# google-research/nerf-from-image

Hardware: AMD Instinct MI355X
Metric: rendered rays/sec (128x128, 64+64 samples) (higher is better)
Workload: dtype f32 (decoder MLP operands split-fp16 hi+lo, 22 bits; strict fp32: config.value_mlp_exact_fp32)

## Files before the change

### include/nfi_hip.h

```cpp
#ifndef NFI_HIP_H
#define NFI_HIP_H

#include <stddef.h>
#include <stdint.h>

#ifdef __cplusplus
extern "C" {
#endif

typedef void* nfi_stream_t;

typedef enum nfi_status {
  NFI_OK = 0,
  NFI_ERR_INVALID_ARGUMENT = -1,
  NFI_ERR_UNSUPPORTED = -2,
  NFI_ERR_WORKSPACE_TOO_SMALL = -3,
  NFI_ERR_LAUNCH = -4
} nfi_status;

enum { NFI_PLANE_CHANNELS = 32, NFI_HIDDEN = 64, NFI_MAX_ATTENTION = 14, NFI_MAX_SAMPLES = 128 };
enum { NFI_MAX_SAMPLES_SINGLE_PASS = 512 };

enum { NFI_TEXEL_F32 = 0, NFI_TEXEL_BF16 = 1, NFI_TEXEL_F16 = 2 };
enum { NFI_TEXELS_PLANAR = 0, NFI_TEXELS_INTERLEAVED = 1 };
// ... 239 lines not shown
  float* semantics;
  float* ray_origins; float* ray_directions; float* near_plane; float* far_plane; uint8_t* hit;
  float* t_coarse; float* sigma_coarse; float* rgb_coarse;
  float* t_fine; float* sigma_fine; float* rgb_fine;
  float* t_sorted; float* weights; int32_t* perm;
  void* workspace; size_t workspace_bytes;
  int skip_missed_rays;
  void* event_start; void* event_stop;
  int tuning;
  void* profile_cycles;
  const float* ray_features;
  float termination_eps;
  int texel_layout;
  void* clock_probe;
  int row_offset; int full_height;
  float* stash_t; float* stash_sigma; float* stash_rgb;
  int rays_ready;
  float* coords;
  float* normals;
} nfi_render_args;
size_t nfi_render_workspace_bytes(int64_t n_rays);
int nfi_render_fwd(const nfi_render_args* a, nfi_stream_t stream);
const char* nfi_render_kernel_name(const nfi_render_args* a);
int nfi_render_setup(const nfi_render_args* a, nfi_stream_t stream);

typedef struct nfi_pnp_args {
  int n_images; int height; int width;
  const float* coords;
  const float* mask;
  float mask_threshold;
  int n_focal; const float* focal_proposals;
  int refine_iterations;
  void* workspace; size_t workspace_bytes;
  float* world2cam;
  float* focal;
  float* error;
} nfi_pnp_args;
size_t nfi_pnp_workspace_bytes(int n_images, int n_focal);
int nfi_pose_pnp(const nfi_pnp_args* a, nfi_stream_t stream);

typedef struct nfi_pose_args {
  int n_images, camera_flipped, normalize_q;
  const float* q; const float* t2; const float* s; const float* z0;
  float* cam2world; float* focal;
  const float* g_cam2world; const float* g_focal;
  float* g_q; float* g_t2; float* g_s; float* g_z0;
// ... 165 lines not shown
```

### nerf_from_image_amd/csrc/nfi_render_host.inc

```

struct RenderWorkspaceHeader {
  uint32_t reduce[3];
  uint32_t counter;
  uint32_t pad[12];
  uint32_t xcd_counter[8][16];
};
static_assert(sizeof(RenderWorkspaceHeader) == 64 + 8 * 64 && offsetof(RenderWorkspaceHeader, xcd_counter) == 64,
              "the render workspace header is read from Python and by the kernels' 16-dword counter stride");

static size_t render_workspace_prefix_bytes(int64_t n_rays) {
  size_t n = (size_t)n_rays;
  return sizeof(RenderWorkspaceHeader) + n * 8 * sizeof(float) + ((n + 63) & ~(size_t)63);
}

static size_t render_workspace_table_offset(int64_t n_rays) {
  return render_workspace_prefix_bytes(n_rays) + kRayBlocks * sizeof(RayPartial);
}

extern "C" size_t nfi_render_workspace_bytes(int64_t n_rays) {
  return render_workspace_table_offset(n_rays) + ((size_t)n_rays / 64) * sizeof(uint32_t);
}

struct BlockGeometry { int shift, ok; uint32_t bw, bh, n_blocks; };
static BlockGeometry render_block_geometry(const nfi_render_args* a) {
  BlockGeometry g;
  const int both = a->width | a->height;
  g.shift = (both & 31) == 0 ? 5 : ((both & 15) == 0 ? 4 : 3);
  const int side = 1 << g.shift;
  g.ok = (a->width % side == 0) && (a->height % side == 0) ? 1 : 0;
  g.bw = (uint32_t)a->width >> g.shift; g.bh = (uint32_t)a->height >> g.shift;
  g.n_blocks = g.bw * g.bh * (uint32_t)a->n_scenes;
  return g;
}

__device__ __forceinline__ uint32_t count_wide_hits(const uint8_t* p, int bytes) {
  uint32_t c = 0;
  if (bytes == 16 && (reinterpret_cast<uintptr_t>(p) & 15) == 0) {
    const uint4 v = *reinterpret_cast<const uint4*>(p);
    c = __popc(v.x & 0x02020202u) + __popc(v.y & 0x02020202u) + __popc(v.z & 0x02020202u) + __popc(v.w & 0x02020202u);
  } else if ((reinterpret_cast<uintptr_t>(p) & 3) == 0) {
    for (int i = 0; i < bytes; i += 4) c += __popc(*reinterpret_cast<const uint32_t*>(p + i) & 0x02020202u);
  } else {
    for (int i = 0; i < bytes; ++i) c += (p[i] >> 1) & 1u;
  }
  return c;
}

struct BlockTableParams { const uint8_t* hit; uint32_t* table; int shift, width, hw; uint32_t bw, bps, n_blocks, groups; };

__global__ __launch_bounds__(256) void raygen_finish_kernel(const RayPartial* __restrict__ partial, int n_partials,
                                                            RenderWorkspaceHeader* __restrict__ head, BlockTableParams t) {
  if (blockIdx.x != 0) {
    __shared__ uint32_t s_part[256], s_count[16];
    const uint32_t G = blockIdx.x - 1, i = threadIdx.x >> 4, sub = threadIdx.x & 15u;
    const uint32_t b = 16u * G + i, scene = b / t.bps, bb = b - scene * t.bps, by = bb / t.bw, bx = bb - by * t.bw;
    const uint8_t* base = t.hit + (size_t)scene * (size_t)t.hw + (size_t)(by << t.shift) * (size_t)t.width + (bx << t.shift);
    const int side = 1 << t.shift, cw = side < 16 ? side : 16, per_row = side / cw;
    uint32_t c = 0;
    for (int ch = (int)sub; ch < side * per_row; ch += 16)
      c += count_wide_hits(base + (size_t)(ch / per_row) * (size_t)t.width + (ch % per_row) * cw, cw);
    s_part[threadIdx.x] = c;
    __syncthreads();
    if (threadIdx.x < 16) {
      uint32_t sum = 0;
      for (int j = 0; j < 16; ++j) sum += s_part[threadIdx.x * 16 + j];
      s_count[threadIdx.x] = sum;
    }
    __syncthreads();
    if (threadIdx.x < 16) {
      const uint32_t me = threadIdx.x, mine = s_count[me];
      uint32_t r = 0;
      for (uint32_t j = 0; j < 16; ++j) r += (s_count[j] > mine || (s_count[j] == mine && j < me)) ? 1u : 0u;
      const uint32_t pair = r < 8 ? r : 15u - r, x = (pair + G) & 7u;
      t.table[16u * G + (r < 8 ? 0u : 8u) + x] = 16u * G + me;
    }
    return;
  }
  uint32_t kmin = 0u, kmax = 0u, cnt = 0u;
  for (int i = threadIdx.x; i < n_partials; i += blockDim.x) {
    const RayPartial p = partial[i];
    kmin = p.kmin > kmin ? p.kmin : kmin;
    kmax = p.kmax > kmax ? p.kmax : kmax;
    cnt += p.cnt;
  }
  block_reduce_keys(kmin, kmax, cnt);
  uint32_t* cells = reinterpret_cast<uint32_t*>(head);
  for (int i = 3 + threadIdx.x; i < (int)(sizeof(RenderWorkspaceHeader) / sizeof(uint32_t)); i += blockDim.x) cells[i] = 0u;
  if (threadIdx.x == 0) { head->reduce[0] = kmin; head->reduce[1] = kmax; head->reduce[2] = cnt; }
  for (uint32_t g = 16u * t.groups + threadIdx.x; g < t.n_blocks; g += blockDim.x) t.table[g] = g;
}

struct RenderWorkspace {
  RenderWorkspaceHeader* head; float* ro; float* rd; float* near_raw; float* far_raw; uint8_t* hit; RayPartial* partial; uint32_t* block_table; int64_t n;
};

static int render_carve(const nfi_render_args* a, RenderWorkspace& w) {
  REQUIRE(a && a->cam2world && a->workspace, "render: null pointer");
  REQUIRE(a->n_scenes > 0 && a->height > 0 && a->width > 0, "render: bad image shape");
  const int64_t n = (int64_t)a->n_scenes * a->height * a->width;
  if (a->workspace_bytes < nfi_render_workspace_bytes(n)) return fail(NFI_ERR_WORKSPACE_TOO_SMALL, "render: workspace too small");
  w.n = n;
  w.head = reinterpret_cast<RenderWorkspaceHeader*>(a->workspace);
  float* rays = reinterpret_cast<float*>(w.head + 1);
  w.ro = a->ray_origins ? a->ray_origins : rays;
  w.rd = a->ray_directions ? a->ray_directions : rays + 3 * n;
  w.near_raw = rays + 6 * n;
  w.far_raw = rays + 7 * n;
  w.hit = a->hit ? a->hit : reinterpret_cast<uint8_t*>(rays + 8 * n);
  w.partial = reinterpret_cast<RayPartial*>(reinterpret_cast<char*>(a->workspace) + render_workspace_prefix_bytes(n));
  w.block_table = reinterpret_cast<uint32_t*>(reinterpret_cast<char*>(a->workspace) + render_workspace_table_offset(n));
  return NFI_OK;
}

static int render_setup(const nfi_render_args* a, const RenderWorkspace& w, hipStream_t s) {
  const int full_h = a->full_height > 0 ? a->full_height : a->height;
  REQUIRE(a->row_offset >= 0 && a->row_offset + a->height <= full_h, "render: row window outside the image");
  CameraParams cam{a->cam2world, a->focal, a->bbox, a->focal ? a->center : nullptr, full_h, a->width, 1, a->height, a->row_offset};
  RaygenOut rout{w.ro, w.rd, w.near_raw, w.far_raw, w.hit, w.partial, a->scene_range};
  const int blocks = (int)std::min<int64_t>((w.n + 255) / 256, kRayBlocks);
  hipLaunchKernelGGL(raygen_kernel, dim3((unsigned)blocks), dim3(256), 0, s, cam, a->n_scenes, rout);
  const BlockGeometry g = render_block_geometry(a);
  const uint32_t n_table = g.ok ? g.n_blocks : (uint32_t)(w.n / 64), groups = g.ok ? g.n_blocks / 16 : 0u;
  const BlockTableParams t{w.hit, w.block_table, g.shift, a->width, a->height * a->width, g.bw, g.bw * g.bh, n_table, groups};
  hipLaunchKernelGGL(raygen_finish_kernel, dim3(1 + groups), dim3(256), 0, s, w.partial, blocks, w.head, t);
  return NFI_OK;
}

extern "C" int nfi_render_setup(const nfi_render_args* a, nfi_stream_t stream) {
  RenderWorkspace w;
  int rc = render_carve(a, w);
  if (rc) return rc;
  rc = render_setup(a, w, (hipStream_t)stream);
  if (rc) return rc;
  return check_launch("render_setup");
}

struct RenderFlags { bool stash, debug_tap, any_tap, strict, term, extra; };

static RenderFlags render_flags(const nfi_render_args* a) {
  RenderFlags f;
  f.stash = a->stash_t || a->stash_sigma || a->stash_rgb;
  f.debug_tap = a->t_coarse || a->sigma_coarse || a->rgb_coarse || a->t_fine || a->sigma_fine || a->rgb_fine ||
                a->t_sorted || a->weights || a->perm || a->near_plane || a->far_plane;
  f.any_tap = f.debug_tap || f.stash;
  f.strict = (a->tuning & NFI_TUNING_EXACT_FP32_MLP) != 0;
  f.term = a->termination_eps > 0.0f;
  f.extra = a->semantics || a->coords || a->normals;
// ... 39 lines not shown
  RenderKernelParams k;
  memset(&k, 0, sizeof(k));
  k.n_scenes = a->n_scenes; k.hw = a->height * a->width; k.S = a->n_samples;
  k.fine = a->fine_sampling; k.white = a->white_background; k.scene_range = a->scene_range;
  k.ro = w.ro; k.rd = w.rd; k.near_raw = w.near_raw; k.far_raw = w.far_raw; k.hit = w.hit; k.reduce = w.head->reduce;
  k.texels = a->texels; k.res = a->plane_res; k.layout = a->texel_layout; k.image = a->decoder_image; k.A = a->n_attention; k.att = a->attention_values;
  k.use_sdf = a->use_sdf; k.beta = a->beta; k.alpha = a->alpha;
  k.noise_c = a->noise_coarse; k.noise_f = a->noise_fine; k.noise_f_stride = a->noise_fine_row_stride;
  k.rgb = a->rgb; k.depth = a->depth; k.mask = a->mask;
  k.near_plane = a->near_plane; k.far_plane = a->far_plane;
  k.t_coarse = a->t_coarse; k.sigma_coarse = a->sigma_coarse; k.rgb_coarse = a->rgb_coarse;
  k.t_fine = a->t_fine; k.sigma_fine = a->sigma_fine; k.rgb_fine = a->rgb_fine;
  k.tap_stride = a->n_samples;
  if (f.stash) {
    k.tap_stride = (a->fine_sampling ? 2 : 1) * a->n_samples; k.stash = 1;
    k.t_coarse = a->stash_t; k.sigma_coarse = a->stash_sigma; k.rgb_coarse = a->stash_rgb;
    if (a->fine_sampling) {
      k.t_fine = a->stash_t + a->n_samples;
      k.sigma_fine = a->stash_sigma + a->n_samples;
      k.rgb_fine = a->stash_rgb + 3 * (size_t)a->n_samples;
    }
  }
  k.t_sorted = a->t_sorted; k.weights = a->weights; k.perm = a->perm;
  k.skip_missed = (a->skip_missed_rays && !f.debug_tap) ? 1 : 0;

  k.counter = &w.head->counter;
  k.xcd_counter = &w.head->xcd_counter[0][0];
  k.width = a->width;
  k.fetch_batch = 2;
  const BlockGeometry geo = render_block_geometry(a);
  k.xcd_block_shift = geo.shift;
  k.xcd_blocks = (!(a->tuning & NFI_TUNING_SINGLE_WORK_COUNTER) && geo.ok) ? 1 : 0;
  k.block_table = (k.xcd_blocks && !(a->tuning & NFI_TUNING_XCD_BLOCKS_IN_ORDER)) ? w.block_table : nullptr;
  const uint32_t bw = geo.bw, bh = geo.bh;
  k.div_scene_rays = make_fastdiv((uint32_t)k.hw * (uint32_t)std::max(a->views_per_scene, 1));
  k.div_bw = make_fastdiv(bw > 0 ? bw : 1u);
  k.div_bps = make_fastdiv(bw * bh > 0 ? bw * bh : 1u);
  k.tile_order = (!(a->tuning & NFI_TUNING_SCANLINE_ORDER) && (a->width % 8 == 0) && (a->height % 8 == 0)) ? 1 : 0;
  k.prof = (unsigned long long*)a->profile_cycles;
  k.xray = a->ray_features;
  k.clock_probe = reinterpret_cast<unsigned long long*>(a->clock_probe);
  k.term_eps = a->termination_eps;
  k.semantics = a->semantics; k.coords = a->coords; k.normals = a->normals;
  return k;
}

using RenderKernel = void (*)(RenderKernelParams);
struct RenderLaunch {
  RenderKernel kernel;
  const char* name;
  int occ;
  size_t max_lds;
  int (*raise_lds)(size_t, const char*);
};
static constexpr char kFwdFamily[] = "render_fwd_kernel", kWideFamily[] = "render_fwd_wide_kernel", kLongFamily[] = "render_fwd_long_kernel";
template <int TEX, bool ATT, int OCC, int MODE, int PREC, bool VD = false>
static RenderLaunch fwd_launch(size_t max_lds = 0) {
  constexpr auto kernel = &render_fwd_kernel<TEX, ATT, OCC, MODE, PREC, VD>;
  return {kernel, KernelName<kFwdFamily, TEX, ATT, OCC, MODE, PREC, VD>::value.s, OCC, max_lds, &ensure_dynamic_lds<kernel>};
}
// ... 95 lines not shown
```

### nerf_from_image_amd/csrc/nfi_render_kernels.inc

```

struct RenderKernelParams {
  int n_scenes, hw, S;
  int fine, white;
  float scene_range;
  const float* ro; const float* rd; const float* near_raw; const float* far_raw; const uint8_t* hit;
  const uint32_t* reduce;
  uint32_t* counter;
  int width;
  int tile_order;
  int xcd_blocks;
  uint32_t* xcd_counter;
  int xcd_block_shift;
  int fetch_batch;
  const uint32_t* block_table;
  const void* texels; int res; int layout;
  const float* image; int A; const float* att;
  int use_sdf; const float* beta; const float* alpha;
  const float* noise_c; const float* noise_f; int64_t noise_f_stride;
  float* rgb; float* depth; float* mask;
  float* near_plane; float* far_plane;
  float* t_coarse; float* sigma_coarse; float* rgb_coarse;
  float* t_fine; float* sigma_fine; float* rgb_fine;
  float* t_sorted; float* weights; int32_t* perm;
  int skip_missed;
  unsigned long long* prof;
  const float* xray;
  float term_eps;
  float* semantics;
  float* coords;
  float* normals;
  unsigned long long* clock_probe;
  FastDiv div_scene_rays, div_bps, div_bw;
  int tap_stride;
  int stash;
};

struct ClockProbe {
  unsigned long long c0 = 0, r0 = 0;
  bool on = false;
  __device__ __forceinline__ void start(const RenderKernelParams& k) {
    on = k.clock_probe && blockIdx.x == 0 && threadIdx.x == 0;
    if (on) { c0 = __builtin_readcyclecounter(); r0 = __builtin_amdgcn_s_memrealtime(); }
  }
  __device__ __forceinline__ void stop(const RenderKernelParams& k) const {
    if (on) {
      k.clock_probe[0] = __builtin_readcyclecounter() - c0;
      k.clock_probe[1] = __builtin_amdgcn_s_memrealtime() - r0;
    }
  }
};

typedef __attribute__((address_space(4))) const RenderKernelParams RenderKernelArgs;
__device__ __forceinline__ RenderKernelArgs* kernel_args_here() {
  auto* p = reinterpret_cast<RenderKernelArgs*>(reinterpret_cast<uintptr_t>(__builtin_amdgcn_kernarg_segment_ptr()));
  asm volatile("" : "+s"(p));
  return p;
}

__device__ __forceinline__ float uniform_f32(float v) {
  return bits2f((uint32_t)__builtin_amdgcn_readfirstlane((int)f2bits(v)));
}

struct RayInputs {
  float ox, oy, oz, dx, dy, dz, near, far, noise, u;
  uint32_t hit;
};

struct RayQueue {
  const RenderKernelParams& k;
  int lane;
  uint32_t n_rays, xcd, bsh, bw, bps, n_blocks, q_cur, pos_next, pos_end, batch, tiles_x;
  uint32_t tab_g, tab_b = 0u, nxt_g = 0xffffffffu, nxt_b = 0u;
  bool dry;
  __device__ __forceinline__ RayQueue(const RenderKernelParams& kk, int l) : k(kk), lane(l) {
    n_rays = (uint32_t)k.n_scenes * (uint32_t)k.hw;
    xcd = k.xcd_blocks ? (__builtin_amdgcn_s_getreg(6164) & 7u) : 0u;
    bsh = (uint32_t)k.xcd_block_shift;
    bw = (uint32_t)k.width >> bsh;
    bps = bw * (((uint32_t)k.hw / (uint32_t)k.width) >> bsh);
    n_blocks = bps * (uint32_t)k.n_scenes;
    q_cur = xcd; pos_next = 0; pos_end = 0; dry = false;
    tab_g = xcd - 8u;
    batch = (uint32_t)k.fetch_batch;
    tiles_x = (uint32_t)k.width >> 3;
  }
  __device__ __forceinline__ uint32_t table_entry(uint32_t g) const {
    typedef __attribute__((address_space(4))) const uint32_t const_u32;
    const uint32_t e = (g | 15u) < n_blocks ? g ^ 8u : g;
    return *reinterpret_cast<const_u32*>(reinterpret_cast<uintptr_t>(k.block_table) + (uintptr_t)e * 4u);
  }
  __device__ __forceinline__ void table_prefetch() {
    if (!k.block_table) return;
    const uint32_t g = tab_g + 8u;
    if (g < n_blocks && g != nxt_g) { nxt_g = g; nxt_b = table_entry(g); }
  }
  __device__ __forceinline__ void table_pin() {
    if (k.block_table) asm volatile("" : "+s"(nxt_b));
  }
  __device__ __forceinline__ uint32_t block_at(uint32_t g) {
    if (!k.block_table) return g;
    if (g != tab_g) {
      tab_b = g == nxt_g ? nxt_b : table_entry(g);
      tab_g = g;
    }
    return tab_b;
  }
  __device__ __forceinline__ uint32_t ray_at(uint32_t q, uint32_t pos) {
    const uint32_t b = block_at((uint32_t)__builtin_amdgcn_readfirstlane((int)((pos >> (2 * bsh)) * 8u + q)));
    const uint32_t in = pos & ((1u << (2 * bsh)) - 1u), scene = fastdiv(b, k.div_bps), bb = b - scene * bps;
    const uint32_t by = fastdiv(bb, k.div_bw), bx = bb - by * bw;
    const uint32_t st = in >> 6, sty = st >> (bsh - 3), stx = st & ((1u << (bsh - 3)) - 1u);
    const uint32_t y = (by << bsh) + (sty << 3) + ((in >> 3) & 7u), x = (bx << bsh) + (stx << 3) + (in & 7u);
    return scene * (uint32_t)k.hw + y * (uint32_t)k.width + x;
  }
  __device__ __forceinline__ uint32_t fetch() {
    if (!k.xcd_blocks) {
      uint32_t p = 0;
      if (lane == 0) p = atomicAdd(k.counter, 1u);
      return (uint32_t)__builtin_amdgcn_readfirstlane((int)p);
    }
    if (pos_next == pos_end && !dry) {
      dry = true;
      table_prefetch();
      for (uint32_t i = 0; i < 8; ++i) {
        uint32_t base = 0;
        if (lane == 0) base = atomicAdd(k.xcd_counter + q_cur * 16, batch);
        if (i == 0) table_pin();
        base = (uint32_t)__builtin_amdgcn_readfirstlane((int)base);
        if ((base >> (2 * bsh)) * 8u + q_cur < n_blocks) { pos_next = base; pos_end = base + batch; dry = false; break; }
        q_cur = (q_cur + 1) & 7u;
      }
    }
    if (dry) return n_rays;
    return ray_at(q_cur, pos_next++);
  }
  __device__ __forceinline__ bool claimed() const { return pos_next != pos_end; }
  __device__ __forceinline__ uint32_t take() { return ray_at(q_cur, pos_next++); }
  __device__ __forceinline__ uint32_t claim_issue() {
    uint32_t raw = 0, off = k.xcd_blocks ? q_cur * 16 : 0;
    asm volatile("" : "+v"(off));
    if (k.xcd_blocks && (claimed() || dry)) return raw;
    table_prefetch();
    if (lane == 0) raw = atomicAdd((k.xcd_blocks ? k.xcd_counter : k.counter) + off, k.xcd_blocks ? batch : 1u);
    table_pin();
    return raw;
  }
  __device__ __forceinline__ uint32_t claim_finish(uint32_t raw) {
    const uint32_t base = (uint32_t)__builtin_amdgcn_readfirstlane((int)raw);
    if (!k.xcd_blocks) return base;
    if (!claimed() && !dry) {
      if ((base >> (2 * bsh)) * 8u + q_cur < n_blocks) { pos_next = base; pos_end = base + batch; }
      else q_cur = (q_cur + 1) & 7u;
    }
    return fetch();
  }
  __device__ __forceinline__ uint32_t ray_of(uint32_t pos) const {
    if (k.xcd_blocks || !k.tile_order) return pos;
    const uint32_t scene = pos / (uint32_t)k.hw, p = pos - scene * (uint32_t)k.hw;
    const uint32_t tile = p >> 6, in = p & 63u;
    const uint32_t ty = tile / tiles_x, tx = tile - ty * tiles_x;
    return scene * (uint32_t)k.hw + ((ty << 3) + (in >> 3)) * (uint32_t)k.width + (tx << 3) + (in & 7u);
  }
};

constexpr int kRenderPlain = 0, kRenderTaps = 1, kRenderProf = 2, kRenderTerm = 3, kRenderExtra = 4, kRenderNormals = 5;
constexpr int kSemPitch = 2 * 64 + 4;
constexpr int kSemPitchWide = 2 * 128 + 8;
extern __shared__ __attribute__((aligned(16))) float nfi_dyn_lds[];

typedef __attribute__((address_space(3))) float lds_float;

template <int NS, class Slab>
__device__ __forceinline__ void composite_coords(const Slab& slab, const float (&w)[NS], int n, int lane, float ox, float oy,
                                                 float oz, float dx, float dy, float dz, float* out3) {
  float cx = 0.0f, cy = 0.0f, cz = 0.0f;
#pragma unroll
  for (int j = 0; j < NS; ++j) {
    const int e = j * 64 + lane;
    if (e < n) {
      const float t = slab.srt[0][e];
      cx += w[j] * (ox + dx * t); cy += w[j] * (oy + dy * t); cz += w[j] * (oz + dz * t);
    }
  }
// ... 60 lines not shown
  if (k.coords && lane < 3) k.coords[(size_t)ray * 3 + lane] = 0.0f;
  if (k.semantics && lane < k.A) k.semantics[(size_t)ray * k.A + lane] = 0.0f;
  if (NRM && lane < 3) k.normals[(size_t)ray * 3 + lane] = bg;
}

__device__ __forceinline__ void zero_stash_row(const RenderKernelParams& k, uint32_t ray, int S, int lane) {
  for (int e = lane; e < S; e += 64) {
    const size_t zs = (size_t)ray * (size_t)k.tap_stride + e;
    k.t_coarse[zs] = 0.0f; k.sigma_coarse[zs] = 0.0f;
    float* q = k.rgb_coarse + zs * 3; q[0] = 0.0f; q[1] = 0.0f; q[2] = 0.0f;
    if (k.fine) {
      k.t_fine[zs] = 0.0f; k.sigma_fine[zs] = 0.0f;
      q = k.rgb_fine + zs * 3; q[0] = 0.0f; q[1] = 0.0f; q[2] = 0.0f;
    }
  }
}

template <bool EXTRA, bool NRM, bool TAPS>
__device__ __forceinline__ void put_missed_ray(const RenderKernelParams& k, uint32_t ray, int S, int lane, float bg) {
  if (lane == 0) store_pixel(k, ray, bg, bg, bg, 0.0f, 0.0f);
  if constexpr (EXTRA) zero_missed_maps<NRM>(k, ray, lane, bg);
  if constexpr (TAPS) {
    if (k.stash) zero_stash_row(k, ray, S, lane);
  }
}

__device__ __forceinline__ uint32_t hit_bytes_scalar(const RenderKernelParams& k, uint32_t ra, uint32_t rb) {
  typedef __attribute__((address_space(4))) const uint32_t const_u32;
  const uintptr_t pa = reinterpret_cast<uintptr_t>(k.hit) + (uint32_t)__builtin_amdgcn_readfirstlane((int)ra),
                  pb = reinterpret_cast<uintptr_t>(k.hit) + (uint32_t)__builtin_amdgcn_readfirstlane((int)rb);
  uint32_t wa = *reinterpret_cast<const_u32*>(pa & ~(uintptr_t)3), wb = *reinterpret_cast<const_u32*>(pb & ~(uintptr_t)3);
  asm volatile("" : "+s"(wa), "+s"(wb));
  return ((wa >> ((uint32_t)(pa & 3) * 8u)) & 0xffu) | (((wb >> ((uint32_t)(pb & 3) * 8u)) & 0xffu) << 8);
}

template <bool EXTRA, bool NRM, bool TAPS, class Load>
__device__ __forceinline__ void skip_miss_run(RayQueue& queue, const RenderKernelParams& k, int S, int lane, float bg,
                                              uint32_t& cur, uint32_t& nxt, Load&& load) {
  put_missed_ray<EXTRA, NRM, TAPS>(k, queue.ray_of(cur), S, lane, bg);
  uint32_t a = nxt;
  while (a < queue.n_rays) {
    const bool two = queue.claimed();
    const uint32_t b = two ? queue.take() : a;
    const uint32_t ra = queue.ray_of(a), rb = queue.ray_of(b);
    const uint32_t hits = hit_bytes_scalar(k, ra, rb);
    uint32_t claim;
// ... 58 lines not shown
      wave_lds_fence();
    }
  }

  auto load_inputs = [&](uint32_t ray, RayInputs& in, auto together) {
    RenderKernelArgs& a = *kernel_args_here();
    const uint8_t* hit = a.hit;
    const float *ro = a.ro, *rd = a.rd, *near_raw = a.near_raw, *far_raw = a.far_raw, *noise_c = a.noise_c, *noise_f = a.noise_f;
    int64_t noise_f_stride = a.noise_f_stride;
    int n_samples = a.S, fine = a.fine;
    if constexpr (decltype(together)::value)
      asm volatile("" : "+s"(hit), "+s"(ro), "+s"(rd), "+s"(near_raw), "+s"(far_raw), "+s"(noise_c), "+s"(noise_f),
                        "+s"(noise_f_stride), "+s"(n_samples), "+s"(fine));
    const size_t r3 = (size_t)ray * 3;
    const bool has = lane < n_samples;
    in.hit = hit[ray];
    in.ox = ro[r3]; in.oy = ro[r3 + 1]; in.oz = ro[r3 + 2];
    in.dx = rd[r3]; in.dy = rd[r3 + 1]; in.dz = rd[r3 + 2];
    in.near = near_raw[ray]; in.far = far_raw[ray];
    in.noise = (noise_c && has) ? noise_c[(size_t)ray * n_samples + lane] : 0.0f;
    in.u = (fine && has) ? noise_f[(size_t)ray * noise_f_stride + lane] : 0.0f;
  };

  RayQueue queue(k, lane);
  auto fetch = [&]() -> uint32_t { return queue.fetch(); };
  uint32_t cur = fetch(), nxt = fetch(), fly = 0;
  RayInputs in, pre;
  unsigned long long pc[12] = {0, 0, 0, 0, 0, 0, 0, 0, 0, 0, 0, 0};
  unsigned long long tk0 = PROF ? __builtin_readcyclecounter() : 0;
  if (cur < n_rays) load_inputs(queue.ray_of(cur), in, std::false_type());
  auto skip_run = [&]() {
    if (k.skip_missed && cur < n_rays && !((uint32_t)__builtin_amdgcn_readfirstlane((int)in.hit) & 2))
      skip_miss_run<EXTRA, NRM, TAPS>(queue, k, S, lane, bg, cur, nxt, [&](uint32_t r) { load_inputs(r, in, std::false_type()); });
  };
  skip_run();
  while (cur < n_rays) {
    if (nxt < n_rays) load_inputs(queue.ray_of(nxt), pre, std::true_type());
    const uint32_t ray = queue.ray_of(cur);
    const uint32_t hitb = in.hit;
    float out_r = bg, out_g = bg, out_b = bg, out_d = 0.0f, out_m = 0.0f;
    unsigned long long t0 = PROF ? __builtin_readcyclecounter() : 0;
    RenderKernelArgs& ka = *kernel_args_here();
    const int scene = (int)fastdiv(ray, FastDiv{ka.div_scene_rays.mul, ka.div_scene_rays.shift});
    if (scene != cur_scene) {
      cur_scene = scene;
      enter_scene<TEX>(P, k, vf, scene, lane);
// ... 150 lines not shown
  WaveSlabWide& slab = slabs[wave];
  float* vf = vfs[wave];
  const int S = k.S;
  const float fill_near = ordered_key_inv(~k.reduce[0]), fill_far = ordered_key_inv(k.reduce[1]);
  const float bg = k.white ? 1.0f : 0.0f;
  const uint32_t n_rays = (uint32_t)k.n_scenes * (uint32_t)k.hw;
  FieldParams P = make_field_params(k.texels, k.res, TEX, k.A, k.use_sdf, k.beta, k.alpha, lds, kImg, k.layout);
  P.vf = vf;
  P.w1t = nfi_dyn_lds; P.w2r0 = nfi_dyn_lds + kW1TFloats;
  int cur_scene = -1;
  typedef __attribute__((address_space(3))) unsigned short lds_u16;
  float* semT = nullptr;
  if constexpr (SEMP != 0) {
    if (k.semantics) {
      semT = reinterpret_cast<float*>(reinterpret_cast<unsigned short*>(nfi_dyn_lds + (NRM ? kNrmLdsFloats : 0)) +
                                      wave * (k.A * kSemPitchWide));
      for (int i = lane; i < k.A * kSemPitchWide / 2; i += 64) ((lds_float*)semT)[i] = 0.0f;
      wave_lds_fence();
    }
  }
  auto sem_col = [&](int c) -> float* {
    return semT ? reinterpret_cast<float*>(reinterpret_cast<unsigned short*>(semT) + c) : nullptr;
  };
  RayQueue queue(k, lane);
  uint32_t cur = queue.fetch(), nxt = 0;
  while (cur < n_rays) {
    nxt = queue.fetch();
    const uint32_t ray = queue.ray_of(cur);
    const uint32_t hitb = k.hit[ray];
    if (k.skip_missed && !(hitb & 2)) {
      if (lane == 0) store_pixel(k, ray, bg, bg, bg, 0.0f, 0.0f);
      if constexpr (EXTRA) zero_missed_maps<NRM>(k, ray, lane, bg);
      if constexpr (TAPS) {
        if (k.stash) zero_stash_row(k, ray, S, lane);
      }
    } else {
      const int scene = (int)fastdiv(ray, k.div_scene_rays);
      if (scene != cur_scene) {
        cur_scene = scene;
        enter_scene<TEX>(P, k, vf, scene, lane);
      }
      const size_t r3 = (size_t)ray * 3;
      const float ox = k.ro[r3], oy = k.ro[r3 + 1], oz = k.ro[r3 + 2];
      const float dx = k.rd[r3], dy = k.rd[r3 + 1], dz = k.rd[r3 + 2];
      float near = k.near_raw[ray], far = k.far_raw[ray];
      finish_planes((hitb & 1) != 0, fill_near, fill_far, near, far);
// ... 162 lines not shown
```

### nerf_from_image_amd/csrc/nfi_render_long.inc

```

struct __attribute__((aligned(16))) WaveSlabLong {
  float srt[5][NFI_MAX_SAMPLES_SINGLE_PASS];
  float stage[16 * 36];
};

template <int TEX, bool ATT, int PREC, bool VD = false>
__global__ __launch_bounds__(256, NFI_RENDER_OCC) void render_fwd_long_kernel(RenderKernelParams k) {
  constexpr int kImg = VD ? kVdImageFloats : kLdsImageFloats;
  constexpr int NS = NFI_MAX_SAMPLES_SINGLE_PASS / 64;
  __shared__ __attribute__((aligned(16))) float lds[kImg];
  __shared__ __attribute__((aligned(16))) float vfs[4][64];
  __shared__ WaveSlabLong slabs[4];
  ClockProbe clock;
  clock.start(k);
  stage_decoder_image<PREC, kImg>(lds, k.image);
  const int lane = lane_id();
  const int wave = threadIdx.x >> 6;
  WaveSlabLong& slab = slabs[wave];
  float* vf = vfs[wave];
  const int S = k.S;
  const int slots = (S + 63) >> 6;
  const float fill_near = ordered_key_inv(~k.reduce[0]), fill_far = ordered_key_inv(k.reduce[1]);
  const float bg = k.white ? 1.0f : 0.0f;
  const uint32_t n_rays = (uint32_t)k.n_scenes * (uint32_t)k.hw;
  FieldParams P = make_field_params(k.texels, k.res, TEX, k.A, k.use_sdf, k.beta, k.alpha, lds, kImg, k.layout);
  P.vf = vf;
  int cur_scene = -1;
  RayQueue queue(k, lane);
  uint32_t cur = queue.fetch(), nxt = 0;
  while (cur < n_rays) {
    nxt = queue.fetch();
    const uint32_t ray = queue.ray_of(cur);
    const uint32_t hitb = k.hit[ray];
    const size_t ts = (size_t)ray * (size_t)k.tap_stride;
    if (k.skip_missed && !(hitb & 2)) {
      if (lane == 0) store_pixel(k, ray, bg, bg, bg, 0.0f, 0.0f);
      if (k.stash) zero_stash_row(k, ray, S, lane);
    } else {
      const int scene = (int)fastdiv(ray, k.div_scene_rays);
      if (scene != cur_scene) {
        cur_scene = scene;
        enter_scene<TEX>(P, k, vf, scene, lane);
      }
      const size_t r3 = (size_t)ray * 3;
      const float ox = k.ro[r3], oy = k.ro[r3 + 1], oz = k.ro[r3 + 2];
      const float dx = k.rd[r3], dy = k.rd[r3 + 1], dz = k.rd[r3 + 2];
      float near = k.near_raw[ray], far = k.far_raw[ray];
      finish_planes((hitb & 1) != 0, fill_near, fill_far, near, far);
      const float dnorm = norm3(dx, dy, dz);
      const size_t rs = (size_t)ray * S;
// ... 33 lines not shown
```

Before: 165.0 million.

## Skip fully-missed 8x8 sub-tiles in the block work queue using per-block live masks

The block-table setup kernel now records, for each screen block, a bitmask of 8x8 sub-tiles that contain at least one ray hit, together with the block's pixel origin. The table entries are widened to 64 bits so the render kernels no longer divide to recover block coordinates. The ray queue maps claim positions only onto live sub-tiles, and when a claim lands in the dead tail of a block it jumps the counter past that block with atomicMax. Dead sub-tiles are filled with background in a separate pass at kernel start, so waves spend no time on rays that miss everything. The cost is more complex queue logic, reclaim loops, extra atomics and an added preamble pass over all blocks.

```diff
diff --git a/include/nfi_hip.h b/include/nfi_hip.h
--- a/include/nfi_hip.h
+++ b/include/nfi_hip.h
@@ -285,6 +285,8 @@
 size_t nfi_render_workspace_bytes(int64_t n_rays);
 int nfi_render_fwd(const nfi_render_args* a, nfi_stream_t stream);
 const char* nfi_render_kernel_name(const nfi_render_args* a);
+int nfi_render_handout_model(uint32_t first_mask, int n_masks, int block_shift, uint32_t slot, int32_t* pixel_of_position,
+                             uint32_t* jump_target);
 int nfi_render_setup(const nfi_render_args* a, nfi_stream_t stream);
 
 typedef struct nfi_pnp_args {
diff --git a/nerf_from_image_amd/csrc/nfi_render_host.inc b/nerf_from_image_amd/csrc/nfi_render_host.inc
--- a/nerf_from_image_amd/csrc/nfi_render_host.inc
+++ b/nerf_from_image_amd/csrc/nfi_render_host.inc
@@ -17,8 +17,12 @@
   return render_workspace_prefix_bytes(n_rays) + kRayBlocks * sizeof(RayPartial);
 }
 
+static size_t render_workspace_entries_offset(int64_t n_rays) {
+  return (render_workspace_table_offset(n_rays) + ((size_t)n_rays / 64) * sizeof(uint32_t) + 7) & ~(size_t)7;
+}
+
 extern "C" size_t nfi_render_workspace_bytes(int64_t n_rays) {
-  return render_workspace_table_offset(n_rays) + ((size_t)n_rays / 64) * sizeof(uint32_t);
+  return render_workspace_entries_offset(n_rays) + 2 * ((size_t)n_rays / 64) * 2 * sizeof(uint32_t);
 }
 
 struct BlockGeometry { int shift, ok; uint32_t bw, bh, n_blocks; };
@@ -33,46 +37,67 @@
   return g;
 }
 
-__device__ __forceinline__ uint32_t count_wide_hits(const uint8_t* p, int bytes) {
-  uint32_t c = 0;
+__device__ __forceinline__ uint2 count_wide_hits(const uint8_t* p, int bytes) {
+  uint2 c = make_uint2(0u, 0u);
   if (bytes == 16 && (reinterpret_cast<uintptr_t>(p) & 15) == 0) {
     const uint4 v = *reinterpret_cast<const uint4*>(p);
-    c = __popc(v.x & 0x02020202u) + __popc(v.y & 0x02020202u) + __popc(v.z & 0x02020202u) + __popc(v.w & 0x02020202u);
+    c.x = __popc(v.x & 0x02020202u) + __popc(v.y & 0x02020202u);
+    c.y = __popc(v.z & 0x02020202u) + __popc(v.w & 0x02020202u);
   } else if ((reinterpret_cast<uintptr_t>(p) & 3) == 0) {
-    for (int i = 0; i < bytes; i += 4) c += __popc(*reinterpret_cast<const uint32_t*>(p + i) & 0x02020202u);
+    for (int i = 0; i < bytes; i += 4) (i < 8 ? c.x : c.y) += __popc(*reinterpret_cast<const uint32_t*>(p + i) & 0x02020202u);
   } else {
-    for (int i = 0; i < bytes; ++i) c += (p[i] >> 1) & 1u;
+    for (int i = 0; i < bytes; ++i) (i < 8 ? c.x : c.y) += (p[i] >> 1) & 1u;
   }
   return c;
 }
 
-struct BlockTableParams { const uint8_t* hit; uint32_t* table; int shift, width, hw; uint32_t bw, bps, n_blocks, groups; };
+struct BlockTableParams {
+  const uint8_t* hit; uint32_t* table; uint32_t* live_by_block; uint32_t* live_by_slot;
+  int shift, width, hw, ok; uint32_t bw, bps, n_blocks, groups;
+};
 
 __global__ __launch_bounds__(256) void raygen_finish_kernel(const RayPartial* __restrict__ partial, int n_partials,
                                                             RenderWorkspaceHeader* __restrict__ head, BlockTableParams t) {
   if (blockIdx.x != 0) {
-    __shared__ uint32_t s_part[256], s_count[16];
+    __shared__ uint32_t s_part[256], s_live[256], s_count[16], s_mask[16];
     const uint32_t G = blockIdx.x - 1, i = threadIdx.x >> 4, sub = threadIdx.x & 15u;
     const uint32_t b = 16u * G + i, scene = b / t.bps, bb = b - scene * t.bps, by = bb / t.bw, bx = bb - by * t.bw;
     const uint8_t* base = t.hit + (size_t)scene * (size_t)t.hw + (size_t)(by << t.shift) * (size_t)t.width + (bx << t.shift);
     const int side = 1 << t.shift, cw = side < 16 ? side : 16, per_row = side / cw;
-    uint32_t c = 0;
-    for (int ch = (int)sub; ch < side * per_row; ch += 16)
-      c += count_wide_hits(base + (size_t)(ch / per_row) * (size_t)t.width + (ch % per_row) * cw, cw);
-    s_part[threadIdx.x] = c;
+    uint32_t c = 0, live = 0;
+    if (b < t.n_blocks) {
+      for (int ch = (int)sub; ch < side * per_row; ch += 16) {
+        const int row = ch / per_row, col = (ch % per_row) * cw;
+        const uint2 h = count_wide_hits(base + (size_t)row * (size_t)t.width + col, cw);
+        const uint32_t st = ((uint32_t)(row >> 3) << (t.shift - 3)) + (uint32_t)(col >> 3);
+        c += h.x + h.y;
+        live |= (h.x ? 1u << st : 0u) | (h.y ? 2u << st : 0u);
+      }
+    }
+    s_part[threadIdx.x] = c; s_live[threadIdx.x] = live;
     __syncthreads();
     if (threadIdx.x < 16) {
-      uint32_t sum = 0;
-      for (int j = 0; j < 16; ++j) sum += s_part[threadIdx.x * 16 + j];
-      s_count[threadIdx.x] = sum;
+      uint32_t sum = 0, mask = 0;
+      for (int j = 0; j < 16; ++j) { sum += s_part[threadIdx.x * 16 + j]; mask |= s_live[threadIdx.x * 16 + j]; }
+      s_count[threadIdx.x] = sum; s_mask[threadIdx.x] = mask;
     }
     __syncthreads();
-    if (threadIdx.x < 16) {
-      const uint32_t me = threadIdx.x, mine = s_count[me];
-      uint32_t r = 0;
-      for (uint32_t j = 0; j < 16; ++j) r += (s_count[j] > mine || (s_count[j] == mine && j < me)) ? 1u : 0u;
-      const uint32_t pair = r < 8 ? r : 15u - r, x = (pair + G) & 7u;
-      t.table[16u * G + (r < 8 ? 0u : 8u) + x] = 16u * G + me;
+    if (threadIdx.x < 16 && 16u * G + threadIdx.x < t.n_blocks) {
+      const uint32_t me = threadIdx.x, mine = s_count[me], mb = 16u * G + me;
+      const uint32_t ms = mb / t.bps, mbb = mb - ms * t.bps, mby = mbb / t.bw, mbx = mbb - mby * t.bw;
+      const uint2 entry = make_uint2((mb & 0xffffu) | (s_mask[me] << 16),
+                                     ms * (uint32_t)t.hw + (mby << t.shift) * (uint32_t)t.width + (mbx << t.shift));
+      uint32_t slot = 16u * G + me, turn = slot;
+      if (G < t.groups) {
+        uint32_t r = 0;
+        for (uint32_t j = 0; j < 16; ++j) r += (s_count[j] > mine || (s_count[j] == mine && j < me)) ? 1u : 0u;
+        const uint32_t pair = r < 8 ? r : 15u - r, x = (pair + G) & 7u;
+        slot = 16u * G + (r < 8 ? 0u : 8u) + x;
+        turn = slot ^ 8u;
+      }
+      t.table[slot] = 16u * G + me;
+      reinterpret_cast<uint2*>(t.live_by_slot)[turn] = entry;
+      reinterpret_cast<uint2*>(t.live_by_block)[16u * G + me] = entry;
     }
     return;
   }
@@ -87,11 +112,18 @@
   uint32_t* cells = reinterpret_cast<uint32_t*>(head);
   for (int i = 3 + threadIdx.x; i < (int)(sizeof(RenderWorkspaceHeader) / sizeof(uint32_t)); i += blockDim.x) cells[i] = 0u;
   if (threadIdx.x == 0) { head->reduce[0] = kmin; head->reduce[1] = kmax; head->reduce[2] = cnt; }
-  for (uint32_t g = 16u * t.groups + threadIdx.x; g < t.n_blocks; g += blockDim.x) t.table[g] = g;
+  if (!t.ok)
+    for (uint32_t g = threadIdx.x; g < t.n_blocks; g += blockDim.x) {
+      t.table[g] = g;
+      const uint2 entry = make_uint2((g & 0xffffu) | 0xffff0000u, 0u);
+      reinterpret_cast<uint2*>(t.live_by_block)[g] = entry;
+      reinterpret_cast<uint2*>(t.live_by_slot)[g] = entry;
+    }
 }
 
 struct RenderWorkspace {
-  RenderWorkspaceHeader* head; float* ro; float* rd; float* near_raw; float* far_raw; uint8_t* hit; RayPartial* partial; uint32_t* block_table; int64_t n;
+  RenderWorkspaceHeader* head; float* ro; float* rd; float* near_raw; float* far_raw; uint8_t* hit; RayPartial* partial;
+  uint32_t* block_table; uint32_t* live_by_block; uint32_t* live_by_slot; int64_t n;
 };
 
 static int render_carve(const nfi_render_args* a, RenderWorkspace& w) {
@@ -109,6 +141,8 @@
   w.hit = a->hit ? a->hit : reinterpret_cast<uint8_t*>(rays + 8 * n);
   w.partial = reinterpret_cast<RayPartial*>(reinterpret_cast<char*>(a->workspace) + render_workspace_prefix_bytes(n));
   w.block_table = reinterpret_cast<uint32_t*>(reinterpret_cast<char*>(a->workspace) + render_workspace_table_offset(n));
+  w.live_by_block = reinterpret_cast<uint32_t*>(reinterpret_cast<char*>(a->workspace) + render_workspace_entries_offset(n));
+  w.live_by_slot = w.live_by_block + 2 * (n / 64);
   return NFI_OK;
 }
 
@@ -121,8 +155,31 @@
   hipLaunchKernelGGL(raygen_kernel, dim3((unsigned)blocks), dim3(256), 0, s, cam, a->n_scenes, rout);
   const BlockGeometry g = render_block_geometry(a);
   const uint32_t n_table = g.ok ? g.n_blocks : (uint32_t)(w.n / 64), groups = g.ok ? g.n_blocks / 16 : 0u;
-  const BlockTableParams t{w.hit, w.block_table, g.shift, a->width, a->height * a->width, g.bw, g.bw * g.bh, n_table, groups};
-  hipLaunchKernelGGL(raygen_finish_kernel, dim3(1 + groups), dim3(256), 0, s, w.partial, blocks, w.head, t);
+  const uint32_t behind = g.ok && n_table > 16u * groups ? 1u : 0u;
+  const BlockTableParams t{w.hit, w.block_table, w.live_by_block, w.live_by_slot, g.shift, a->width, a->height * a->width, g.ok,
+                           g.bw, g.bw * g.bh, n_table, groups};
+  hipLaunchKernelGGL(raygen_finish_kernel, dim3(1 + groups + behind), dim3(256), 0, s, w.partial, blocks, w.head, t);
+  return NFI_OK;
+}
+
+extern "C" int nfi_render_handout_model(uint32_t first_mask, int n_masks, int block_shift, uint32_t slot,
+                                        int32_t* pixel_of_position, uint32_t* jump_target) {
+  REQUIRE(pixel_of_position && jump_target, "render_handout_model: null pointer");
+  REQUIRE(block_shift >= 3 && block_shift <= 5 && n_masks >= 0, "render_handout_model: block_shift must be 3, 4 or 5");
+  const uint32_t bsh = (uint32_t)block_shift, positions = 1u << (2 * bsh);
+  REQUIRE((uint64_t)first_mask + (uint64_t)n_masks <= (1ull << (positions / 64u)) && slot < (1u << (31 - 2 * bsh)),
+          "render_handout_model: masks have one bit per 8x8 sub-tile of the block; slot * positions must stay below 2^31");
+  for (int m = 0; m < n_masks; ++m)
+    for (uint32_t in = 0; in < positions; ++in) {
+      const uint32_t mask = first_mask + (uint32_t)m, pos = slot * positions + in;
+      const size_t cell = (size_t)m * positions + in;
+      jump_target[cell] = LiveMask::jump_target(bsh, pos);
+      pixel_of_position[cell] = -1;
+      if (LiveMask::dead_tail(mask, bsh, pos)) continue;
+      uint32_t y, x;
+      LiveMask::pixel_in_block(LiveMask::subtile_of_rank(mask, in >> 6), in, bsh, y, x);
+      pixel_of_position[cell] = (int32_t)((y << bsh) + x);
+    }
   return NFI_OK;
 }
 
@@ -208,20 +265,19 @@
     }
   }
   k.t_sorted = a->t_sorted; k.weights = a->weights; k.perm = a->perm;
-  k.skip_missed = (a->skip_missed_rays && !f.debug_tap) ? 1 : 0;
+  k.skip_missed = (a->skip_missed_rays && !f.debug_tap) ? kSkipMissed : 0;
 
   k.counter = &w.head->counter;
   k.xcd_counter = &w.head->xcd_counter[0][0];
   k.width = a->width;
-  k.fetch_batch = 2;
   const BlockGeometry geo = render_block_geometry(a);
   k.xcd_block_shift = geo.shift;
   k.xcd_blocks = (!(a->tuning & NFI_TUNING_SINGLE_WORK_COUNTER) && geo.ok) ? 1 : 0;
-  k.block_table = (k.xcd_blocks && !(a->tuning & NFI_TUNING_XCD_BLOCKS_IN_ORDER)) ? w.block_table : nullptr;
-  const uint32_t bw = geo.bw, bh = geo.bh;
+  k.block_table = !k.xcd_blocks ? nullptr : ((a->tuning & NFI_TUNING_XCD_BLOCKS_IN_ORDER) ? w.live_by_block : w.live_by_slot);
+  k.live_by_block = w.live_by_block;
+  k.n_blocks = geo.n_blocks;
+  if (k.xcd_blocks && k.skip_missed) k.skip_missed |= kSkipLiveMasks;
   k.div_scene_rays = make_fastdiv((uint32_t)k.hw * (uint32_t)std::max(a->views_per_scene, 1));
-  k.div_bw = make_fastdiv(bw > 0 ? bw : 1u);
-  k.div_bps = make_fastdiv(bw * bh > 0 ? bw * bh : 1u);
   k.tile_order = (!(a->tuning & NFI_TUNING_SCANLINE_ORDER) && (a->width % 8 == 0) && (a->height % 8 == 0)) ? 1 : 0;
   k.prof = (unsigned long long*)a->profile_cycles;
   k.xray = a->ray_features;
diff --git a/nerf_from_image_amd/csrc/nfi_render_kernels.inc b/nerf_from_image_amd/csrc/nfi_render_kernels.inc
--- a/nerf_from_image_amd/csrc/nfi_render_kernels.inc
+++ b/nerf_from_image_amd/csrc/nfi_render_kernels.inc
@@ -11,7 +11,6 @@
   int xcd_blocks;
   uint32_t* xcd_counter;
   int xcd_block_shift;
-  int fetch_batch;
   const uint32_t* block_table;
   const void* texels; int res; int layout;
   const float* image; int A; const float* att;
@@ -30,9 +29,36 @@
   float* coords;
   float* normals;
   unsigned long long* clock_probe;
-  FastDiv div_scene_rays, div_bps, div_bw;
+  FastDiv div_scene_rays;
   int tap_stride;
   int stash;
+  const uint32_t* live_by_block;
+  uint32_t n_blocks;
+};
+
+constexpr int kSkipMissed = 1, kSkipLiveMasks = 2;
+
+struct LiveMask {
+  static __host__ __device__ __forceinline__ uint32_t live_length(uint32_t mask) { return 64u * (uint32_t)__builtin_popcount(mask); }
+  static __host__ __device__ __forceinline__ uint32_t subtile_of_rank(uint32_t mask, uint32_t r) {
+    uint32_t st = 0u, c = (uint32_t)__builtin_popcount(mask & 0xffu);
+    if (r >= c) { st += 8u; r -= c; mask >>= 8; }
+    c = (uint32_t)__builtin_popcount(mask & 0xfu);
+    if (r >= c) { st += 4u; r -= c; mask >>= 4; }
+    c = (uint32_t)__builtin_popcount(mask & 3u);
+    if (r >= c) { st += 2u; r -= c; mask >>= 2; }
+    return st + (r >= (mask & 1u) ? 1u : 0u);
+  }
+  static __host__ __device__ __forceinline__ bool dead_tail(uint32_t mask, uint32_t bsh, uint32_t pos) {
+    return (pos & ((1u << (2 * bsh)) - 1u)) >= live_length(mask);
+  }
+  static __host__ __device__ __forceinline__ uint32_t jump_target(uint32_t bsh, uint32_t pos) {
+    return ((pos >> (2 * bsh)) + 1u) << (2 * bsh);
+  }
+  static __host__ __device__ __forceinline__ void pixel_in_block(uint32_t st, uint32_t in, uint32_t bsh, uint32_t& y, uint32_t& x) {
+    const uint32_t sty = st >> (bsh - 3), stx = st & ((1u << (bsh - 3)) - 1u);
+    y = (sty << 3) + ((in >> 3) & 7u); x = (stx << 3) + (in & 7u);
+  }
 };
 
 struct ClockProbe {
@@ -40,7 +66,7 @@
   bool on = false;
   __device__ __forceinline__ void start(const RenderKernelParams& k) {
     on = k.clock_probe && blockIdx.x == 0 && threadIdx.x == 0;
-    if (on) { c0 = __builtin_readcyclecounter(); r0 = __builtin_amdgcn_s_memrealtime(); }
+    if (k.clock_probe) { c0 = __builtin_readcyclecounter(); r0 = __builtin_amdgcn_s_memrealtime(); }
   }
   __device__ __forceinline__ void stop(const RenderKernelParams& k) const {
     if (on) {
@@ -69,96 +95,113 @@
 struct RayQueue {
   const RenderKernelParams& k;
   int lane;
-  uint32_t n_rays, xcd, bsh, bw, bps, n_blocks, q_cur, pos_next, pos_end, batch, tiles_x;
-  uint32_t tab_g, tab_b = 0u, nxt_g = 0xffffffffu, nxt_b = 0u;
-  bool dry;
+  static constexpr uint32_t batch = 2u, kNone = 0xffffffffu;
+  uint32_t n_rays, xcd, bsh, n_blocks, q_cur, pos_next;
+  uint32_t tab_g, tab_b = 0u, tab_o = 0u, nxt_b = 0u, nxt_o = 0u;
+  static constexpr uint32_t kDry = 8u;
+  __device__ __forceinline__ bool dry() const { return (q_cur & kDry) != 0u; }
   __device__ __forceinline__ RayQueue(const RenderKernelParams& kk, int l) : k(kk), lane(l) {
     n_rays = (uint32_t)k.n_scenes * (uint32_t)k.hw;
     xcd = k.xcd_blocks ? (__builtin_amdgcn_s_getreg(6164) & 7u) : 0u;
     bsh = (uint32_t)k.xcd_block_shift;
-    bw = (uint32_t)k.width >> bsh;
-    bps = bw * (((uint32_t)k.hw / (uint32_t)k.width) >> bsh);
-    n_blocks = bps * (uint32_t)k.n_scenes;
-    q_cur = xcd; pos_next = 0; pos_end = 0; dry = false;
+    n_blocks = k.n_blocks;
+    q_cur = xcd; pos_next = kNone;
     tab_g = xcd - 8u;
-    batch = (uint32_t)k.fetch_batch;
-    tiles_x = (uint32_t)k.width >> 3;
-  }
-  __device__ __forceinline__ uint32_t table_entry(uint32_t g) const {
-    typedef __attribute__((address_space(4))) const uint32_t const_u32;
-    const uint32_t e = (g | 15u) < n_blocks ? g ^ 8u : g;
-    return *reinterpret_cast<const_u32*>(reinterpret_cast<uintptr_t>(k.block_table) + (uintptr_t)e * 4u);
+  }
+  __device__ __forceinline__ uint2 table_entry(uint32_t g) const {
+    typedef __attribute__((address_space(4))) const uint64_t const_u64;
+    const uint64_t e = *reinterpret_cast<const_u64*>(reinterpret_cast<uintptr_t>(k.block_table) + (uintptr_t)g * 8u);
+    return make_uint2((uint32_t)e, (uint32_t)(e >> 32));
   }
   __device__ __forceinline__ void table_prefetch() {
+    nxt_b = 0u; nxt_o = 0u;
     if (!k.block_table) return;
     const uint32_t g = tab_g + 8u;
-    if (g < n_blocks && g != nxt_g) { nxt_g = g; nxt_b = table_entry(g); }
+    if (g < n_blocks) { const uint2 e = table_entry(g); nxt_b = e.x; nxt_o = e.y; }
   }
   __device__ __forceinline__ void table_pin() {
-    if (k.block_table) asm volatile("" : "+s"(nxt_b));
-  }
-  __device__ __forceinline__ uint32_t block_at(uint32_t g) {
-    if (!k.block_table) return g;
+    if (k.block_table) asm volatile("" : "+s"(nxt_b), "+s"(nxt_o));
+  }
+  __device__ __forceinline__ uint32_t block_at(uint32_t g, bool fresh) {
     if (g != tab_g) {
-      tab_b = g == nxt_g ? nxt_b : table_entry(g);
+      if (fresh && g == tab_g + 8u) { tab_b = nxt_b; tab_o = nxt_o; }
+      else { const uint2 e = table_entry(g); tab_b = e.x; tab_o = e.y; }
       tab_g = g;
     }
     return tab_b;
   }
   __device__ __forceinline__ uint32_t ray_at(uint32_t q, uint32_t pos) {
-    const uint32_t b = block_at((uint32_t)__builtin_amdgcn_readfirstlane((int)((pos >> (2 * bsh)) * 8u + q)));
-    const uint32_t in = pos & ((1u << (2 * bsh)) - 1u), scene = fastdiv(b, k.div_bps), bb = b - scene * bps;
-    const uint32_t by = fastdiv(bb, k.div_bw), bx = bb - by * bw;
-    const uint32_t st = in >> 6, sty = st >> (bsh - 3), stx = st & ((1u << (bsh - 3)) - 1u);
-    const uint32_t y = (by << bsh) + (sty << 3) + ((in >> 3) & 7u), x = (bx << bsh) + (stx << 3) + (in & 7u);
-    return scene * (uint32_t)k.hw + y * (uint32_t)k.width + x;
+    const uint32_t e = block_at((uint32_t)__builtin_amdgcn_readfirstlane((int)((pos >> (2 * bsh)) * 8u + q)), false);
+    const uint32_t in = pos & ((1u << (2 * bsh)) - 1u);
+    uint32_t st = in >> 6, y, x;
+    if (k.skip_missed & kSkipLiveMasks) st = LiveMask::subtile_of_rank(e >> 16, st);
+    LiveMask::pixel_in_block(st, in, bsh, y, x);
+    return tab_o + y * (uint32_t)k.width + x;
+  }
+  __device__ __forceinline__ bool dead_claim(uint32_t base) {
+    const uint32_t e = block_at((base >> (2 * bsh)) * 8u + q_cur, true);
+    if (!(k.skip_missed & kSkipLiveMasks)) return false;
+    if (!LiveMask::dead_tail(e >> 16, bsh, base)) return false;
+    if (lane == 0) atomicMax(k.xcd_counter + q_cur * 16, LiveMask::jump_target(bsh, base));
+    return true;
   }
   __device__ __forceinline__ uint32_t fetch() {
-    if (!k.xcd_blocks) {
+    if (!k.block_table) {
       uint32_t p = 0;
       if (lane == 0) p = atomicAdd(k.counter, 1u);
       return (uint32_t)__builtin_amdgcn_readfirstlane((int)p);
     }
-    if (pos_next == pos_end && !dry) {
-      dry = true;
+    if (pos_next == kNone && !dry()) {
+      bool found = false;
       table_prefetch();
-      for (uint32_t i = 0; i < 8; ++i) {
-        uint32_t base = 0;
-        if (lane == 0) base = atomicAdd(k.xcd_counter + q_cur * 16, batch);
-        if (i == 0) table_pin();
-        base = (uint32_t)__builtin_amdgcn_readfirstlane((int)base);
-        if ((base >> (2 * bsh)) * 8u + q_cur < n_blocks) { pos_next = base; pos_end = base + batch; dry = false; break; }
-        q_cur = (q_cur + 1) & 7u;
-      }
-    }
-    if (dry) return n_rays;
-    return ray_at(q_cur, pos_next++);
-  }
-  __device__ __forceinline__ bool claimed() const { return pos_next != pos_end; }
-  __device__ __forceinline__ uint32_t take() { return ray_at(q_cur, pos_next++); }
+      const uint32_t reclaims = ((n_blocks + 7u) >> 3) + 2u;
+      for (uint32_t i = 0; i < 8 && !found; ++i) {
+        for (uint32_t t = 0; t < reclaims; ++t) {
+          uint32_t base = 0;
+          if (lane == 0) base = atomicAdd(k.xcd_counter + q_cur * 16, batch);
+          table_pin();
+          base = (uint32_t)__builtin_amdgcn_readfirstlane((int)base);
+          if ((base >> (2 * bsh)) * 8u + q_cur >= n_blocks) break;
+          if (!dead_claim(base)) { pos_next = base; found = true; break; }
+          table_prefetch();
+        }
+        if (!found) q_cur = (q_cur + 1) & 7u;
+      }
+      if (!found) q_cur |= kDry;
+    }
+    if (dry()) return n_rays;
+    return take();
+  }
+  __device__ __forceinline__ bool claimed() const { return pos_next != kNone; }
+  __device__ __forceinline__ uint32_t take() {
+    const uint32_t pos = pos_next;
+    pos_next = (pos & 1u) ? kNone : pos + 1u;
+    return ray_at(q_cur, pos);
+  }
   __device__ __forceinline__ uint32_t claim_issue() {
-    uint32_t raw = 0, off = k.xcd_blocks ? q_cur * 16 : 0;
+    uint32_t raw = 0, off = k.block_table ? q_cur * 16 : 0;
     asm volatile("" : "+v"(off));
-    if (k.xcd_blocks && (claimed() || dry)) return raw;
+    if (k.block_table && (claimed() || dry())) return raw;
     table_prefetch();
-    if (lane == 0) raw = atomicAdd((k.xcd_blocks ? k.xcd_counter : k.counter) + off, k.xcd_blocks ? batch : 1u);
+    if (lane == 0) raw = atomicAdd((k.block_table ? k.xcd_counter : k.counter) + off, k.block_table ? batch : 1u);
     table_pin();
     return raw;
   }
   __device__ __forceinline__ uint32_t claim_finish(uint32_t raw) {
     const uint32_t base = (uint32_t)__builtin_amdgcn_readfirstlane((int)raw);
-    if (!k.xcd_blocks) return base;
-    if (!claimed() && !dry) {
-      if ((base >> (2 * bsh)) * 8u + q_cur < n_blocks) { pos_next = base; pos_end = base + batch; }
-      else q_cur = (q_cur + 1) & 7u;
+    if (!k.block_table) return base;
+    if (!claimed() && !dry()) {
+      if ((base >> (2 * bsh)) * 8u + q_cur < n_blocks) {
+        if (!dead_claim(base)) pos_next = base;
+      } else q_cur = (q_cur + 1) & 7u;
     }
     return fetch();
   }
   __device__ __forceinline__ uint32_t ray_of(uint32_t pos) const {
-    if (k.xcd_blocks || !k.tile_order) return pos;
+    if (k.block_table || !k.tile_order) return pos;
     const uint32_t scene = pos / (uint32_t)k.hw, p = pos - scene * (uint32_t)k.hw;
     const uint32_t tile = p >> 6, in = p & 63u;
-    const uint32_t ty = tile / tiles_x, tx = tile - ty * tiles_x;
+    const uint32_t tiles_x = (uint32_t)k.width >> 3, ty = tile / tiles_x, tx = tile - ty * tiles_x;
     return scene * (uint32_t)k.hw + ((ty << 3) + (in >> 3)) * (uint32_t)k.width + (tx << 3) + (in & 7u);
   }
 };
@@ -265,6 +308,33 @@
   if constexpr (EXTRA) zero_missed_maps<NRM>(k, ray, lane, bg);
   if constexpr (TAPS) {
     if (k.stash) zero_stash_row(k, ray, S, lane);
+  }
+}
+
+template <bool EXTRA, bool NRM, bool TAPS>
+__device__ __forceinline__ void put_dead_subtiles(const RenderKernelParams& k, int S, int lane, float bg) {
+  if (!(k.skip_missed & kSkipLiveMasks)) return;
+  const uint32_t bsh = (uint32_t)k.xcd_block_shift;
+  const uint32_t all = (1u << (1u << (2 * (bsh - 3)))) - 1u, wave = threadIdx.x >> 6, waves = blockDim.x >> 6;
+  for (uint32_t b = blockIdx.x; b < k.n_blocks; b += gridDim.x) {
+    const uint32_t origin = k.live_by_block[2u * b + 1u];
+    uint32_t dead = ~(k.live_by_block[2u * b] >> 16) & all;
+    for (uint32_t i = 0; dead; dead &= dead - 1u, ++i) {
+      if (i % waves != wave) continue;
+      uint32_t y, x;
+      LiveMask::pixel_in_block((uint32_t)__builtin_ctz(dead), 0u, bsh, y, x);
+      const uint32_t ray0 = origin + y * (uint32_t)k.width + x;
+      store_pixel(k, ray0 + (uint32_t)(lane >> 3) * (uint32_t)k.width + (uint32_t)(lane & 7), bg, bg, bg, 0.0f, 0.0f);
+      if constexpr (EXTRA || TAPS) {
+        for (uint32_t p = 0; p < 64u; ++p) {
+          const uint32_t ray = ray0 + (p >> 3) * (uint32_t)k.width + (p & 7u);
+          if constexpr (EXTRA) zero_missed_maps<NRM>(k, ray, lane, bg);
+          if constexpr (TAPS) {
+            if (k.stash) zero_stash_row(k, ray, S, lane);
+          }
+        }
+      }
+    }
   }
 }
 
@@ -369,6 +439,7 @@
     in.u = (fine && has) ? noise_f[(size_t)ray * noise_f_stride + lane] : 0.0f;
   };
 
+  put_dead_subtiles<EXTRA, NRM, TAPS>(k, S, lane, bg);
   RayQueue queue(k, lane);
   auto fetch = [&]() -> uint32_t { return queue.fetch(); };
   uint32_t cur = fetch(), nxt = fetch(), fly = 0;
@@ -565,6 +636,7 @@
   auto sem_col = [&](int c) -> float* {
     return semT ? reinterpret_cast<float*>(reinterpret_cast<unsigned short*>(semT) + c) : nullptr;
   };
+  put_dead_subtiles<EXTRA, NRM, TAPS>(k, S, lane, bg);
   RayQueue queue(k, lane);
   uint32_t cur = queue.fetch(), nxt = 0;
   while (cur < n_rays) {
diff --git a/nerf_from_image_amd/csrc/nfi_render_long.inc b/nerf_from_image_amd/csrc/nfi_render_long.inc
--- a/nerf_from_image_amd/csrc/nfi_render_long.inc
+++ b/nerf_from_image_amd/csrc/nfi_render_long.inc
@@ -26,6 +26,7 @@
   FieldParams P = make_field_params(k.texels, k.res, TEX, k.A, k.use_sdf, k.beta, k.alpha, lds, kImg, k.layout);
   P.vf = vf;
   int cur_scene = -1;
+  put_dead_subtiles<false, false, true>(k, S, lane, bg);
   RayQueue queue(k, lane);
   uint32_t cur = queue.fetch(), nxt = 0;
   while (cur < n_rays) {
```

Measured after the change: 166.5 million (median of 6 runs). About the same (+0.9%).
